# Zokrates/ZoKrates

Measured on NVIDIA H100. Metric: groth16_constraints_per_sec, higher is better.
Workload: dtype u256-montgomery

## Files before the change

zokrates_b200/csrc/ntt_tile.cuh:

```cuda
#pragma once
#include "ntt.cuh"
#include "rt.cuh"

#if !defined(ZKB_EMU)
namespace zkb {

static constexpr uint32_t NTT2_PLANE = NTT_TILE;
static constexpr uint32_t NTT2_SMEM = (2 * NTT2_PLANE + 2 * 512) * 16;

__device__ __forceinline__ uint32_t ntt2_slot(uint32_t pos) {
  const uint32_t x = ((pos >> 3) & 1u) * 2u ^ ((pos >> 4) & 1u) * 5u ^ ((pos >> 5) & 1u) * 6u;
  return pos ^ x;
}
__device__ __forceinline__ uint32_t ntt2_wslot(uint32_t wi) {
  const uint32_t x = ((wi >> 3) & 1u) * 3u ^ ((wi >> 4) & 1u) * 6u ^ ((wi >> 5) & 1u) * 7u ^ ((wi >> 6) & 1u) * 5u ^ ((wi >> 7) & 1u) * 1u ^
                     ((wi >> 8) & 1u) * 2u;
  return wi ^ x;
}

template <class Fr>
__device__ __forceinline__ Fr ntt2_ld(const uint4* lo, const uint4* hi, uint32_t slot) {
  static_assert(sizeof(Fr) == 32, "two 16-byte halves");
  Fr r;
  uint4 a = lo[slot], b = hi[slot];
  r.v[0] = a.x; r.v[1] = a.y; r.v[2] = a.z; r.v[3] = a.w;
  r.v[4] = b.x; r.v[5] = b.y; r.v[6] = b.z; r.v[7] = b.w;
  return r;
}
template <class Fr>
__device__ __forceinline__ void ntt2_st(uint4* lo, uint4* hi, uint32_t slot, const Fr& r) {
  lo[slot] = make_uint4(r.v[0], r.v[1], r.v[2], r.v[3]);
  hi[slot] = make_uint4(r.v[4], r.v[5], r.v[6], r.v[7]);
}
template <class Fr>
__device__ __forceinline__ Fr ntt2_ldg(const Fr* p) {
  const uint4 a = __ldg((const uint4*)p), b = __ldg((const uint4*)p + 1);
  Fr r;
  r.v[0] = a.x; r.v[1] = a.y; r.v[2] = a.z; r.v[3] = a.w;
  r.v[4] = b.x; r.v[5] = b.y; r.v[6] = b.z; r.v[7] = b.w;
  return r;
}
__device__ __forceinline__ void ntt2_cp_async16(void* smem_dst, const void* gmem_src) {
  const uint32_t s = (uint32_t)__cvta_generic_to_shared(smem_dst);
  asm volatile("cp.async.cg.shared.global [%0], [%1], 16;" ::"r"(s), "l"(gmem_src) : "memory");
}
__device__ __forceinline__ void ntt2_cp_async_wait() { asm volatile("cp.async.wait_all;" ::: "memory"); }

template <class Fr>
__device__ __forceinline__ Fr ntt2_factor(const Fr* tw, const NttPass& ps, uint32_t low, uint32_t j_local) {
  const uint32_t k1 = __brev(j_local) >> (32 - ps.S);
  const uint32_t e = (low * k1) << (ps.log_n - ps.lo_bit - ps.S);
  const uint32_t half = 1u << (ps.log_n - 1);
  Fr f = ntt2_ldg<Fr>(tw + (e & (half - 1)));
  return (e & half) ? Fr::neg(f) : f;
}

template <class Fr, bool DIT, int K>
__device__ __forceinline__ void ntt2_stages(Fr* __restrict__ x, const Fr* __restrict__ tw, const Fr* __restrict__ scale, const NttPass& ps, uint4* dlo, uint4* dhi, const uint4* wlo,
                                            const uint4* whi, uint32_t tile, uint32_t done, bool first, bool last) {
  constexpr uint32_t R = 1u << K;
  const uint32_t G = NTT_TILE >> ps.S;
  const uint32_t lg_hmin = DIT ? done : ps.S - done - K;
  const uint32_t hmin = 1u << lg_hmin;
  const uint32_t per_group = (1u << ps.S) >> K;
  uint32_t low_base = 0;
  if (ps.lo_bit) low_base = (tile % ((1u << ps.lo_bit) / G)) * G;
  for (uint32_t tt = threadIdx.x; tt < (NTT_TILE >> K); tt += NTT_BLOCK) {
    uint32_t g, jj;
    if (ps.lo_bit) { g = tt % G; jj = tt / G; } else { jj = tt % per_group; g = tt / per_group; }
    const uint32_t off = jj & (hmin - 1), blk = jj >> lg_hmin;
    const uint32_t j0 = (blk << (lg_hmin + K)) | off;
    const uint32_t low = ps.lo_bit ? low_base + g : 0;
    Fr e[R];
#pragma unroll
    for (uint32_t m = 0; m < R; m++) {
      const uint32_t j = j0 + m * hmin;
      e[m] = ntt2_ld<Fr>(dlo, dhi, ntt2_slot(ps.lo_bit ? j * G + g : (g << ps.S) + j));
    }
    if (DIT && first) {
      if (ps.lo_bit) {
#pragma unroll
        for (uint32_t m = 0; m < R; m++) if (low) e[m] = Fr::mul(e[m], ntt2_factor<Fr>(tw, ps, low, j0 + m * hmin));
      } else if (scale) {
#pragma unroll
        for (uint32_t m = 0; m < R; m++) {
          uint32_t jd, lw;
          const uint32_t gi = ntt_tile_global(ps, tile, (g << ps.S) + j0 + m * hmin, &jd, &lw);
          e[m] = Fr::mul(e[m], ntt2_ldg<Fr>(scale + bitrev32(gi, ps.log_n)));
        }
      }
    }
    const bool dif_factor = !DIT && last && ps.lo_bit && low;
#pragma unroll
    for (int q = 0; q < K; q++) {
      const uint32_t hm = DIT ? (1u << q) : (1u << (K - 1 - q));
      const uint32_t lg_hl = lg_hmin + (DIT ? q : K - 1 - q);
#pragma unroll
      for (uint32_t m = 0; m < R; m++) {
        if (m & hm) continue;
        const uint32_t imod = off + (m & (hm - 1)) * hmin;
        const uint32_t wi = imod << (9 - lg_hl);
        Fr u = e[m];
        if (DIT) {
          Fr v = wi ? Fr::mul(e[m + hm], ntt2_ld<Fr>(wlo, whi, ntt2_wslot(wi))) : e[m + hm];
          e[m] = Fr::add(u, v);
          e[m + hm] = Fr::sub(u, v);
        } else {
          Fr v = e[m + hm];
          e[m] = Fr::add(u, v);
          Fr d = Fr::sub(u, v);
          e[m + hm] = wi ? Fr::mul(d, ntt2_ld<Fr>(wlo, whi, ntt2_wslot(wi))) : d;
        }
      }
    }
    if (dif_factor) {
#pragma unroll
      for (uint32_t m = 0; m < R; m++) e[m] = Fr::mul(e[m], ntt2_factor<Fr>(tw, ps, low, j0 + m * hmin));
    }
#pragma unroll
    for (uint32_t m = 0; m < R; m++) {
      const uint32_t j = j0 + m * hmin;
      const uint32_t pos = ps.lo_bit ? j * G + g : (g << ps.S) + j;
      if (last) {
        uint32_t jd, lw;
        x[ntt_tile_global(ps, tile, pos, &jd, &lw)] = e[m];
      } else {
        ntt2_st<Fr>(dlo, dhi, ntt2_slot(pos), e[m]);
      }
    }
  }
}

template <class Fr, bool DIT>
__global__ void __launch_bounds__(NTT_BLOCK, 4) zkb_ntt_tile2(Fr* x_all, const Fr* tw, const Fr* scale, NttPass ps, uint32_t tiles) {
  extern __shared__ uint4 ntt2_smem[];
  uint4* dlo = ntt2_smem;
  uint4* dhi = dlo + NTT2_PLANE;
  uint4* wlo = dhi + NTT2_PLANE;
  uint4* whi = wlo + 512;
  {
    const uint32_t stride = 1u << (ps.log_n - NTT_TILE_LOG);
    for (uint32_t k = threadIdx.x; k < 512; k += NTT_BLOCK) {
      const uint4* src = (const uint4*)(tw + (size_t)k * stride);
      wlo[ntt2_wslot(k)] = src[0];
      whi[ntt2_wslot(k)] = src[1];
    }
  }
  const uint32_t lg_tpv = ps.log_n - NTT_TILE_LOG;
  for (uint32_t bt = blockIdx.x; bt < tiles; bt += gridDim.x) {
    Fr* x = x_all + ((size_t)(bt >> lg_tpv) << ps.log_n);
    const uint32_t tile = bt & ((1u << lg_tpv) - 1u);
    __syncthreads();
    for (uint32_t k = 0; k < NTT_TILE / NTT_BLOCK; k++) {
      const uint32_t e = threadIdx.x + k * NTT_BLOCK;
      uint32_t j, low;
      const uint4* src = (const uint4*)(x + ntt_tile_global(ps, tile, e, &j, &low));
      const uint32_t slot = ntt2_slot(e);
      ntt2_cp_async16(dlo + slot, src);
      ntt2_cp_async16(dhi + slot, src + 1);
    }
    ntt2_cp_async_wait();
    __syncthreads();
    uint32_t done = 0;
    for (uint32_t p = 0; p < ps.nk; p++) {
      const bool first = p == 0, last = p + 1 == ps.nk;
      switch (ps.K[p]) {
        case 3: ntt2_stages<Fr, DIT, 3>(x, tw, scale, ps, dlo, dhi, wlo, whi, tile, done, first, last); break;
        case 2: ntt2_stages<Fr, DIT, 2>(x, tw, scale, ps, dlo, dhi, wlo, whi, tile, done, first, last); break;
        default: ntt2_stages<Fr, DIT, 1>(x, tw, scale, ps, dlo, dhi, wlo, whi, tile, done, first, last); break;
      }
      done += ps.K[p];
      if (!last) __syncthreads();
    }
  }
}

template <class Fr, bool DIT>
inline void launch_ntt_tile2(Stream st, Fr* x, const Fr* tw, const Fr* scale, const NttPass& ps, size_t tiles, int sm_count) {
  static bool configured = false;
  if (!configured) {
    ZKB_CUDA(cudaFuncSetAttribute(zkb_ntt_tile2<Fr, DIT>, cudaFuncAttributeMaxDynamicSharedMemorySize, (int)NTT2_SMEM));
    configured = true;
  }
  launch_counter()++;
  const size_t resident = (size_t)sm_count * 4;
  const unsigned grid = (unsigned)(tiles < resident ? tiles : resident);
  zkb_ntt_tile2<Fr, DIT><<<grid, NTT_BLOCK, NTT2_SMEM, st.s>>>(x, tw, scale, ps, (uint32_t)tiles);
  ZKB_CUDA(cudaGetLastError());
}

}
#endif
```

Before: 52.08 million.

## Double-buffer NTT tile loads and restructure tile kernel into fixed radix-4 phases

The tile NTT kernel now double-buffers the data tile in shared memory, issuing cp.async loads for the next tile while the current one is processed. Each thread handles a fixed unrolled set of butterflies with block size NTT_TILE/4, and the pass schedule is hard-coded as radix-4 phases plus one radix-2 phase when the stage count is odd. Index math moves to shifts, the bank swizzle changes, and twiddle factors are applied one element at a time to limit register pressure. The cost is double the shared memory and fewer resident blocks per SM (2 instead of 4), and passes with fewer than 3 stages are now rejected.

```diff
diff --git a/zokrates_b200/csrc/ntt_tile.cuh b/zokrates_b200/csrc/ntt_tile.cuh
--- a/zokrates_b200/csrc/ntt_tile.cuh
+++ b/zokrates_b200/csrc/ntt_tile.cuh
@@ -6,10 +6,11 @@
 namespace zkb {
 
 static constexpr uint32_t NTT2_PLANE = NTT_TILE;
-static constexpr uint32_t NTT2_SMEM = (2 * NTT2_PLANE + 2 * 512) * 16;
+static constexpr uint32_t NTT2_THREADS = NTT_TILE >> 2;
+static constexpr uint32_t NTT2_SMEM = (2 * 2 * NTT2_PLANE + 2 * 512) * 16;
 
 __device__ __forceinline__ uint32_t ntt2_slot(uint32_t pos) {
-  const uint32_t x = ((pos >> 3) & 1u) * 2u ^ ((pos >> 4) & 1u) * 5u ^ ((pos >> 5) & 1u) * 6u;
+  const uint32_t x = ((pos >> 3) & 1u) * 3u ^ ((pos >> 4) & 1u) * 5u;
   return pos ^ x;
 }
 __device__ __forceinline__ uint32_t ntt2_wslot(uint32_t wi) {
@@ -55,42 +56,56 @@
   return (e & half) ? Fr::neg(f) : f;
 }
 
-template <class Fr, bool DIT, int K>
-__device__ __forceinline__ void ntt2_stages(Fr* __restrict__ x, const Fr* __restrict__ tw, const Fr* __restrict__ scale, const NttPass& ps, uint4* dlo, uint4* dhi, const uint4* wlo,
-                                            const uint4* whi, uint32_t tile, uint32_t done, bool first, bool last) {
+__device__ __forceinline__ uint32_t ntt2_global(const NttPass& ps, uint32_t tile, uint32_t e) {
+  if (ps.lo_bit == 0) return (tile << NTT_TILE_LOG) | e;
+  const uint32_t lg_g = NTT_TILE_LOG - ps.S, lg_per_hi = ps.lo_bit - lg_g;
+  const uint32_t lb = tile & ((1u << lg_per_hi) - 1u);
+  return ((tile >> lg_per_hi) << (ps.lo_bit + ps.S)) | ((e >> lg_g) << ps.lo_bit) | (lb << lg_g) | (e & ((1u << lg_g) - 1u));
+}
+
+extern __shared__ uint4 ntt2_smem[];
+static constexpr uint32_t NTT2_WHI = 512, NTT2_DATA = 1024;
+
+template <class Fr, bool DIT, int K, bool FIRST, bool LAST>
+__device__ __forceinline__ void ntt2_stages(Fr* x_all, const Fr* tw, const Fr* scale, const NttPass& ps,
+                                            uint32_t dbuf, uint32_t bt, uint32_t thread, uint32_t done) {
   constexpr uint32_t R = 1u << K;
-  const uint32_t G = NTT_TILE >> ps.S;
+  const uint32_t lg_tpv = ps.log_n - NTT_TILE_LOG;
+  const uint32_t tile = bt & ((1u << lg_tpv) - 1u);
+  uint4* dlo = ntt2_smem + dbuf;
+  uint4* dhi = dlo + NTT2_PLANE;
+  const uint4* wlo = ntt2_smem;
+  const uint4* whi = ntt2_smem + NTT2_WHI;
+  const uint32_t lg_g = NTT_TILE_LOG - ps.S;
   const uint32_t lg_hmin = DIT ? done : ps.S - done - K;
   const uint32_t hmin = 1u << lg_hmin;
-  const uint32_t per_group = (1u << ps.S) >> K;
+  const uint32_t lg_pg = ps.S - K;
   uint32_t low_base = 0;
-  if (ps.lo_bit) low_base = (tile % ((1u << ps.lo_bit) / G)) * G;
-  for (uint32_t tt = threadIdx.x; tt < (NTT_TILE >> K); tt += NTT_BLOCK) {
+  if (ps.lo_bit) low_base = (tile & ((1u << (ps.lo_bit - lg_g)) - 1u)) << lg_g;
+#pragma unroll
+  for (uint32_t i = 0; i < (NTT_TILE >> K) / NTT2_THREADS; i++) {
+    const uint32_t tt = thread + i * NTT2_THREADS;
     uint32_t g, jj;
-    if (ps.lo_bit) { g = tt % G; jj = tt / G; } else { jj = tt % per_group; g = tt / per_group; }
+    if (ps.lo_bit) { g = tt & ((1u << lg_g) - 1u); jj = tt >> lg_g; } else { jj = tt & ((1u << lg_pg) - 1u); g = tt >> lg_pg; }
     const uint32_t off = jj & (hmin - 1), blk = jj >> lg_hmin;
     const uint32_t j0 = (blk << (lg_hmin + K)) | off;
     const uint32_t low = ps.lo_bit ? low_base + g : 0;
+    const uint32_t pos0 = ps.lo_bit ? (j0 << lg_g) + g : (g << ps.S) + j0;
+    const uint32_t lg_pstep = ps.lo_bit ? lg_hmin + lg_g : lg_hmin;
     Fr e[R];
 #pragma unroll
-    for (uint32_t m = 0; m < R; m++) {
-      const uint32_t j = j0 + m * hmin;
-      e[m] = ntt2_ld<Fr>(dlo, dhi, ntt2_slot(ps.lo_bit ? j * G + g : (g << ps.S) + j));
-    }
-    if (DIT && first) {
-      if (ps.lo_bit) {
-#pragma unroll
-        for (uint32_t m = 0; m < R; m++) if (low) e[m] = Fr::mul(e[m], ntt2_factor<Fr>(tw, ps, low, j0 + m * hmin));
-      } else if (scale) {
-#pragma unroll
-        for (uint32_t m = 0; m < R; m++) {
-          uint32_t jd, lw;
-          const uint32_t gi = ntt_tile_global(ps, tile, (g << ps.S) + j0 + m * hmin, &jd, &lw);
-          e[m] = Fr::mul(e[m], ntt2_ldg<Fr>(scale + bitrev32(gi, ps.log_n)));
-        }
-      }
-    }
-    const bool dif_factor = !DIT && last && ps.lo_bit && low;
+    for (uint32_t m = 0; m < R; m++) e[m] = ntt2_ld<Fr>(dlo, dhi, ntt2_slot(pos0 + (m << lg_pstep)));
+    if (DIT && FIRST && (ps.lo_bit ? low != 0 : scale != nullptr)) {
+#pragma unroll 1
+      for (uint32_t m = 0; m < R; m++) {
+        const Fr f = ps.lo_bit ? ntt2_factor<Fr>(tw, ps, low, j0 + m * hmin)
+                               : ntt2_ldg<Fr>(scale + bitrev32(ntt2_global(ps, tile, pos0 + (m << lg_pstep)), ps.log_n));
+        const Fr t = Fr::mul(e[0], f);
+#pragma unroll
+        for (uint32_t r = 0; r + 1 < R; r++) e[r] = e[r + 1];
+        e[R - 1] = t;
+      }
+    }
 #pragma unroll
     for (int q = 0; q < K; q++) {
       const uint32_t hm = DIT ? (1u << q) : (1u << (K - 1 - q));
@@ -113,65 +128,73 @@
         }
       }
     }
-    if (dif_factor) {
-#pragma unroll
-      for (uint32_t m = 0; m < R; m++) e[m] = Fr::mul(e[m], ntt2_factor<Fr>(tw, ps, low, j0 + m * hmin));
-    }
-#pragma unroll
-    for (uint32_t m = 0; m < R; m++) {
-      const uint32_t j = j0 + m * hmin;
-      const uint32_t pos = ps.lo_bit ? j * G + g : (g << ps.S) + j;
-      if (last) {
-        uint32_t jd, lw;
-        x[ntt_tile_global(ps, tile, pos, &jd, &lw)] = e[m];
-      } else {
-        ntt2_st<Fr>(dlo, dhi, ntt2_slot(pos), e[m]);
-      }
-    }
+    if (!DIT && LAST && low) {
+#pragma unroll 1
+      for (uint32_t m = 0; m < R; m++) {
+        x_all[((size_t)(bt >> lg_tpv) << ps.log_n) + ntt2_global(ps, tile, pos0 + (m << lg_pstep))] =
+            Fr::mul(e[0], ntt2_factor<Fr>(tw, ps, low, j0 + m * hmin));
+#pragma unroll
+        for (uint32_t r = 0; r + 1 < R; r++) e[r] = e[r + 1];
+      }
+    } else {
+#pragma unroll
+      for (uint32_t m = 0; m < R; m++) {
+        const uint32_t pos = pos0 + (m << lg_pstep);
+        if (LAST) x_all[((size_t)(bt >> lg_tpv) << ps.log_n) + ntt2_global(ps, tile, pos)] = e[m];
+        else ntt2_st<Fr>(dlo, dhi, ntt2_slot(pos), e[m]);
+      }
+    }
+  }
+}
+
+__device__ __forceinline__ uint32_t ntt2_phases(uint32_t S) { return (S + 1) >> 1; }
+
+template <class Fr>
+__device__ __forceinline__ void ntt2_load_tile(Fr* x_all, const NttPass& ps, uint32_t bt, uint32_t dbuf, uint32_t thread) {
+  const uint32_t lg_tpv = ps.log_n - NTT_TILE_LOG;
+  const Fr* x = x_all + ((size_t)(bt >> lg_tpv) << ps.log_n);
+  const uint32_t tile = bt & ((1u << lg_tpv) - 1u);
+#pragma unroll
+  for (uint32_t k = 0; k < NTT_TILE / NTT2_THREADS; k++) {
+    const uint32_t e = thread + k * NTT2_THREADS;
+    const uint4* src = (const uint4*)(x + ntt2_global(ps, tile, e));
+    const uint32_t slot = dbuf + ntt2_slot(e);
+    ntt2_cp_async16(ntt2_smem + slot, src);
+    ntt2_cp_async16(ntt2_smem + slot + NTT2_PLANE, src + 1);
   }
 }
 
 template <class Fr, bool DIT>
-__global__ void __launch_bounds__(NTT_BLOCK, 4) zkb_ntt_tile2(Fr* x_all, const Fr* tw, const Fr* scale, NttPass ps, uint32_t tiles) {
-  extern __shared__ uint4 ntt2_smem[];
-  uint4* dlo = ntt2_smem;
-  uint4* dhi = dlo + NTT2_PLANE;
-  uint4* wlo = dhi + NTT2_PLANE;
-  uint4* whi = wlo + 512;
+__global__ void __launch_bounds__(NTT2_THREADS, 2) zkb_ntt_tile2(Fr* x_all, const Fr* tw, const Fr* scale, NttPass ps, uint32_t tiles) {
+  const uint32_t thread = threadIdx.x;
+  uint32_t bt = blockIdx.x;
+  ntt2_load_tile<Fr>(x_all, ps, bt, NTT2_DATA, thread);
   {
-    const uint32_t stride = 1u << (ps.log_n - NTT_TILE_LOG);
-    for (uint32_t k = threadIdx.x; k < 512; k += NTT_BLOCK) {
-      const uint4* src = (const uint4*)(tw + (size_t)k * stride);
-      wlo[ntt2_wslot(k)] = src[0];
-      whi[ntt2_wslot(k)] = src[1];
-    }
-  }
-  const uint32_t lg_tpv = ps.log_n - NTT_TILE_LOG;
-  for (uint32_t bt = blockIdx.x; bt < tiles; bt += gridDim.x) {
-    Fr* x = x_all + ((size_t)(bt >> lg_tpv) << ps.log_n);
-    const uint32_t tile = bt & ((1u << lg_tpv) - 1u);
-    __syncthreads();
-    for (uint32_t k = 0; k < NTT_TILE / NTT_BLOCK; k++) {
-      const uint32_t e = threadIdx.x + k * NTT_BLOCK;
-      uint32_t j, low;
-      const uint4* src = (const uint4*)(x + ntt_tile_global(ps, tile, e, &j, &low));
-      const uint32_t slot = ntt2_slot(e);
-      ntt2_cp_async16(dlo + slot, src);
-      ntt2_cp_async16(dhi + slot, src + 1);
-    }
+    const uint32_t tstride = 1u << (ps.log_n - NTT_TILE_LOG);
+    for (uint32_t k = thread; k < 512; k += NTT2_THREADS) {
+      const uint4* src = (const uint4*)(tw + (size_t)k * tstride);
+      ntt2_smem[ntt2_wslot(k)] = src[0];
+      ntt2_smem[NTT2_WHI + ntt2_wslot(k)] = src[1];
+    }
+  }
+  const uint32_t nk = ntt2_phases(ps.S);
+  for (uint32_t cur = 0; bt < tiles; bt += gridDim.x, cur ^= 1u) {
+    const uint32_t dbuf = NTT2_DATA + cur * (2 * NTT2_PLANE);
     ntt2_cp_async_wait();
     __syncthreads();
-    uint32_t done = 0;
-    for (uint32_t p = 0; p < ps.nk; p++) {
-      const bool first = p == 0, last = p + 1 == ps.nk;
-      switch (ps.K[p]) {
-        case 3: ntt2_stages<Fr, DIT, 3>(x, tw, scale, ps, dlo, dhi, wlo, whi, tile, done, first, last); break;
-        case 2: ntt2_stages<Fr, DIT, 2>(x, tw, scale, ps, dlo, dhi, wlo, whi, tile, done, first, last); break;
-        default: ntt2_stages<Fr, DIT, 1>(x, tw, scale, ps, dlo, dhi, wlo, whi, tile, done, first, last); break;
-      }
-      done += ps.K[p];
-      if (!last) __syncthreads();
-    }
+    if (bt + gridDim.x < tiles)
+      ntt2_load_tile<Fr>(x_all, ps, bt + gridDim.x, NTT2_DATA + (cur ^ 1u) * (2 * NTT2_PLANE), thread);
+    const bool odd = ps.S & 1u;
+    if (DIT && odd) ntt2_stages<Fr, DIT, 1, true, false>(x_all, tw, scale, ps, dbuf, bt, thread, 0);
+    else ntt2_stages<Fr, DIT, 2, true, false>(x_all, tw, scale, ps, dbuf, bt, thread, 0);
+    uint32_t done = (DIT && odd) ? 1 : 2;
+    for (uint32_t p = 1; p + 1 < nk; p++, done += 2) {
+      __syncthreads();
+      ntt2_stages<Fr, DIT, 2, false, false>(x_all, tw, scale, ps, dbuf, bt, thread, done);
+    }
+    __syncthreads();
+    if (!DIT && odd) ntt2_stages<Fr, DIT, 1, false, true>(x_all, tw, scale, ps, dbuf, bt, thread, done);
+    else ntt2_stages<Fr, DIT, 2, false, true>(x_all, tw, scale, ps, dbuf, bt, thread, done);
   }
 }
 
@@ -182,10 +205,11 @@
     ZKB_CUDA(cudaFuncSetAttribute(zkb_ntt_tile2<Fr, DIT>, cudaFuncAttributeMaxDynamicSharedMemorySize, (int)NTT2_SMEM));
     configured = true;
   }
+  if (ps.S < 3) throw Error(ZKB_E_INTERNAL, "tile pass of fewer than 3 stages");
   launch_counter()++;
-  const size_t resident = (size_t)sm_count * 4;
+  const size_t resident = 2 * (size_t)sm_count;
   const unsigned grid = (unsigned)(tiles < resident ? tiles : resident);
-  zkb_ntt_tile2<Fr, DIT><<<grid, NTT_BLOCK, NTT2_SMEM, st.s>>>(x, tw, scale, ps, (uint32_t)tiles);
+  zkb_ntt_tile2<Fr, DIT><<<grid, NTT2_THREADS, NTT2_SMEM, st.s>>>(x, tw, scale, ps, (uint32_t)tiles);
   ZKB_CUDA(cudaGetLastError());
 }
 
```

Result: faster. 53.13 million, median of 6 (+2.0%).
